# qq456cvb/CPPF

Measured on AMD Instinct MI355X. Metric: point-pairs/sec (PPF+MLP+vote+argmax), N=4096 K=128; 1/2/4/8 GPU, higher is better.
Workload: dtype f32; 1 GPU; c2: single object N=4096 K=128 (P=524288 pairs), bottle config, res 0.004, grid 26x76x26, num_rots 72 adaptive, fused PPF+MLP(MFMA f32)+decode of the  ... (full text: bench_full.json); parallelism=objects x1

## Files before the change

### cppf_amd/csrc/pair_mlp.hip

```cpp
#include <hip/hip_runtime.h>
#include <stdint.h>
#include <string.h>

#include "../../include/cppf.h"
#include "cppf_math.h"

using namespace cppf;

typedef float f32x4 __attribute__((ext_vector_type(4)));
typedef float f32x2 __attribute__((ext_vector_type(2)));
typedef float f32x4u __attribute__((ext_vector_type(4), aligned(4)));

#define CPPF_CHECK_LAUNCH()                         \
    do {                                            \
        hipError_t e__ = hipGetLastError();         \
        if (e__ != hipSuccess) return (int)e__;     \
    } while (0)

#include "pair_layout.h"

static bool is_std(int F, const int* dims, int n_res, int out_dim)
{
    return F == STD_F && n_res == 3 && dims[0] == 84 && dims[1] == 32 && dims[2] == 32 && dims[3] == 16 &&
           out_dim >= 1 && out_dim <= 16 * STD_NOB;
// ... 163 lines not shown
    if (__any(u < 0.f)) {
        asm volatile("" ::: "memory");
        int ak = 64;
#pragma unroll
        for (int k = NL - 1; k >= 0; --k)
            if (v[k] == mall) ak = k;
        const int am = NL * g + ak;
        int best = min(am, (int)xor16u((unsigned)am, lane));
        best = min(best, (int)xor32u((unsigned)best, lane));
        if (u < 0.f) { bin = best; owner = am == best; }
    }
    return owner;
}

struct MlpArgs {
    const float* pc;
    const float* nrm;
    const float* feat;
    const void* idxs;
    const float* packed;
    const float* u_tr;
    const float* u_rot;
    const float* table;
    float* out;
    float* outputs;
    float* heads;
    int64_t P;
    int out_dim;
    int idx64;
    float vr0, vr1;
    const int32_t* sel;
    const int32_t* n_sel;
};

template <typename T>
__device__ __forceinline__ const T& at_off(const void* base, unsigned byte_off)
{
    return *reinterpret_cast<const T*>(static_cast<const char*>(base) + byte_off);
}
template <typename T>
__device__ __forceinline__ T& at_off(void* base, unsigned byte_off)
{
    return *reinterpret_cast<T*>(static_cast<char*>(base) + byte_off);
}
__device__ __forceinline__ f3 ld3o(const float* __restrict__ base, int i)
{
    const unsigned o = __umul24((unsigned)i, 12u);
    return {at_off<float>(base, o), at_off<float>(base + 1, o), at_off<float>(base + 2, o)};
}

template <bool SEL>
__device__ __forceinline__ unsigned pair_row(const MlpArgs& A, int slot, int Pn)
{
    const unsigned s = (unsigned)min(slot, Pn - 1);
    return SEL ? (unsigned)at_off<int>(A.sel, s * 4u) : s;
}

template <bool SEL>
__device__ __forceinline__ void load_pair_idx(const MlpArgs& A, int slot, int Pn, int& ia, int& ib)
{
    const unsigned p = pair_row<SEL>(A, slot, Pn);
    const unsigned o = p * (A.idx64 ? 16u : 8u);
    ia = at_off<int>(A.idxs, o);
    ib = at_off<int>(static_cast<const char*>(A.idxs) + (A.idx64 ? 8 : 4), o);
}

__device__ __forceinline__ float ppf_from(f3 pa, f3 pb, f3 na, f3 nb, int g)
{
    const f3 xy = sub3(pa, pb);
    const float d = sqrt_rn((xy.x * xy.x + xy.y * xy.y) + xy.z * xy.z);
    const float den = d + 1e-7f;
    const float rden = refined_rcp(den);
    const f3 u = {div_by(xy.x, den, rden), div_by(xy.y, den, rden), div_by(xy.z, den, rden)};
    const float p0 = (na.x * u.x + na.y * u.y) + na.z * u.z;
    const float p1 = (nb.x * u.x + nb.y * u.y) + nb.z * u.z;
    const float p2 = (na.x * nb.x + na.y * nb.y) + na.z * nb.z;
    (void)g;
    const bool g0 = __builtin_amdgcn_inverse_ballot_w64(0x000000000000ffffull), g1 = __builtin_amdgcn_inverse_ballot_w64(0x00000000ffff0000ull),
               g2 = __builtin_amdgcn_inverse_ballot_w64(0x0000ffff00000000ull);
    const float s23 = g2 ? p2 : d, s123 = g1 ? p1 : s23;
    return g0 ? p0 : s123;
}

#define PROJ_PPB 8
__device__ __forceinline__ void point_proj_body(const float* __restrict__ feat, const float* __restrict__ packed, float* __restrict__ T,
                                                int64_t N)
{
    __shared__ float f[PROJ_PPB][STD_F];
    const int half = threadIdx.x >> 7, r = threadIdx.x & 127;
    const int64_t n0 = (int64_t)blockIdx.x * PROJ_PPB;
    for (int i = threadIdx.x; i < PROJ_PPB * STD_F; i += 256) {
        const int64_t n = n0 + i / STD_F;
        f[i / STD_F][i % STD_F] = n < N ? feat[n * STD_F + i % STD_F] : 0.f;
    }
    __syncthreads();
    float acc[PROJ_PPB / 2];
    const float b = r < 64 ? packed[OFF_BPT + r] : 0.f;
#pragma unroll
    for (int q = 0; q < PROJ_PPB / 2; ++q) acc[q] = b;
#pragma unroll 8
    for (int k = 0; k < STD_F; ++k) {
        const float w = packed[OFF_WPT + k * PROJ_COLS + r];
#pragma unroll
        for (int q = 0; q < PROJ_PPB / 2; ++q) acc[q] = fmaf(w, f[half + 2 * q][k], acc[q]);
    }
#pragma unroll
    for (int q = 0; q < PROJ_PPB / 2; ++q) {
        const int64_t n = n0 + half + 2 * q;
        if (n < N) T[n * PROJ_COLS + r] = acc[q];
    }
}
__global__ __launch_bounds__(256) void point_proj_kernel(const float* __restrict__ feat, const float* __restrict__ packed,
                                                         float* __restrict__ T, int64_t N)
{
    point_proj_body(feat, packed, T, N);
}
struct ProjBatch { const float* feat[8]; const float* packed[8]; float* table[8]; int64_t N[8]; };
__global__ __launch_bounds__(256) void point_proj_batch_kernel(ProjBatch B)
{
    const int i = blockIdx.y;
    if ((int64_t)blockIdx.x * PROJ_PPB >= B.N[i]) return;
    point_proj_body(B.feat[i], B.packed[i], B.table[i], B.N[i]);
}

template <bool LOGITS, bool DECODE, bool HEADS, bool SEL>
__device__ __forceinline__ void pair_mlp_body(const MlpArgs& A, const int wg, const int n_wg)
{
    extern __shared__ __attribute__((aligned(16))) float W[];
    {
        const f32x4* src = reinterpret_cast<const f32x4*>(A.packed);
        f32x4* dst = reinterpret_cast<f32x4*>(W);
        for (int k = threadIdx.x; k < STD_LDS / 4; k += MLP_THREADS) {
            int from = k;
            if (DECODE && k >= OFF_WF / 4 && k < OFF_B0B / 4) from = OFF_WFD / 4 + (k - OFF_WF / 4);
            if (DECODE && k >= OFF_BF / 4) from = OFF_BFD / 4 + (k - OFF_BF / 4);
            dst[k] = src[from];
        }
    }
    float* lut = W + STD_LDS;
    int* tile_ctr = reinterpret_cast<int*>(W + STD_LDS + 112);
    if (threadIdx.x == 0) *tile_ctr = 0;
    if (DECODE && threadIdx.x < 100) {
        const int k = threadIdx.x;
        float v;
        if (k < 32) v = ((float)k / 31.0f * 2.0f) * A.vr0 - A.vr0;
        else if (k < 64) v = (float)(k - 32) / 31.0f * A.vr1;
        else v = (float)(k - 64) / 35.0f * (float)CPPF_PI;
        lut[k] = v;
    }
    __syncthreads();

    const int lane = threadIdx.x & 63;
    const int j = lane & 15, g = lane >> 4;
    __builtin_assume(g >= 0 && g < 4);
    int Pn = (int)A.P;
    if (SEL) Pn = min(max(*A.n_sel, 0), Pn);
    const int n_tiles = (Pn + 16 * PB - 1) / (16 * PB);
    const int per_wg = (n_tiles + n_wg - 1) / n_wg;
    const int wg_begin = wg * per_wg;
    const int wg_end = min(wg_begin + per_wg, n_tiles);
    auto claim = [&]() -> int {
        int v = 0;
        if (lane == 0) v = atomicAdd(tile_ctr, 1);
        return wg_begin + __builtin_amdgcn_readfirstlane(v);
    };
    int cur = claim();
    if (cur >= wg_end) return;
    int nxt = claim();

    f32x4 acc[PB][4];
    int ia1[PB], ib1[PB];
    {
        f32x4 ta[PB][4], tb[PB][4];
        float xp[PB];
        int ia[PB], ib[PB];
#pragma unroll
        for (int pb = 0; pb < PB; ++pb) load_pair_idx<SEL>(A, cur * (16 * PB) + pb * 16 + j, Pn, ia[pb], ib[pb]);
#pragma unroll
        for (int pb = 0; pb < PB; ++pb) {
            const unsigned oa = (unsigned)ia[pb] * (PROJ_COLS * 4u) + 16u * g, ob_ = (unsigned)ib[pb] * (PROJ_COLS * 4u) + 256u + 16u * g;
#pragma unroll
            for (int ob = 0; ob < 4; ++ob) { ta[pb][ob] = at_off<f32x4>(A.table, oa + 64u * ob); tb[pb][ob] = at_off<f32x4>(A.table, ob_ + 64u * ob); }
            xp[pb] = ppf_from(ld3o(A.pc, ia[pb]), ld3o(A.pc, ib[pb]), ld3o(A.nrm, ia[pb]), ld3o(A.nrm, ib[pb]), g);
        }
        const int nt = nxt < wg_end ? nxt : cur;
#pragma unroll
        for (int pb = 0; pb < PB; ++pb) load_pair_idx<SEL>(A, nt * (16 * PB) + pb * 16 + j, Pn, ia1[pb], ib1[pb]);
// ... 654 lines not shown
```

### cppf_amd/csrc/vote.hip

```cpp
#include "vote_common.h"

#define VOTE_MAX_TILES 64
#define VOTE_WIN 72

__host__ __device__ inline int vote_fixed_bits_of(int64_t chunk_pairs, int n_rots)
{
    const double cap = 2048.0 * 4294967296.0 / ((double)(chunk_pairs > 0 ? chunk_pairs : 1) * n_rots) - 4.0;
    int kk = 24;
    while (kk > 8 && (double)(1u << kk) > cap) --kk;
    return kk;
}


static int v3_fixed_bits_bound(int64_t n_ppfs, int n_rots, int gx, int gy, int gz);
static bool v3_eligible(int64_t n_ppfs, int n_rots, int gx, int gy, int gz);
static size_t v3_workspace_bytes(int64_t n_ppfs, int gx, int gy, int gz);
static size_t v3_workspace_bytes_dyn(int many_tiles, int64_t n_ppfs);
static int v3_fused_tiles();
extern "C" int cppf_vote_fixed_point_bits(int64_t n_ppfs, int n_rots, int gx, int gy, int gz)
{
    if (n_rots < 1 || n_rots > CPPF_MAX_ROTS || gx < 1 || gy < 1 || gz < 1 || n_ppfs < 0) return -1;
    return v3_eligible(n_ppfs, n_rots, gx, gy, gz) ? v3_fixed_bits_bound(n_ppfs, n_rots, gx, gy, gz) : 0;
}

// ... 1056 lines not shown
            }
            while (qn >= 64 || (!more && qn > 0)) {
                const int take = qn < 64 ? qn : 64;
                __builtin_amdgcn_fence(__ATOMIC_ACQ_REL, "wavefront");
                const uint32_t off = lane < take ? pairq[qn - take + lane] : 0u;
                qn -= take;
                process(p0 + off, lane < take, 0u, 0u);
            }
            if (!more) break;
        }
    }

#ifdef V3_TRACE
    if (lane == 0) { trace[8 + wave] = wall_clock64(); unsigned hw; asm volatile("s_getreg_b32 %0, hwreg(HW_REG_HW_ID)" : "=s"(hw)); if (wave < 8) trace[24 + wave] = hw; }
#endif
    __syncthreads();
#ifdef V3_TRACE
    if (tid == 0) { trace[2] = wall_clock64(); trace[4] = (unsigned long long)t; trace[5] = (unsigned long long)c; trace[6] = (unsigned long long)ctrl[8]; trace[7] = (unsigned long long)ctrl[9]; }
#endif
    const int slot = v3_slot_words(pt, gz);
    uint4* part4 = reinterpret_cast<uint4*>(A.partials + (int64_t)bid * slot);
    const uint4* t4 = reinterpret_cast<const uint4*>(tile);
    for (int k = tid; k < (nwords + 3) >> 2; k += V3_THREADS) part4[k] = t4[k];
    bool wrote = false;
    auto to_plane = [&](const int w, const int lx, const int ly, const int z) {
        const uint32_t v = tile[w];
        if (v == 0u) return;
        unsigned long long* dst = &A.plane[((int64_t)(x0 + lx) * gy + (y0 + ly)) * gz + z];
        if (S > 0.f) atomicAdd(dst, (unsigned long long)v); else atomicAdd(reinterpret_cast<float*>(dst), __uint_as_float(v));
        wrote = true;
    };
    if (pt.hx && x0 + tx < gx)
        for (int k = tid; k < (ty + 1) * gz && k < ltyz; k += V3_THREADS) { const int ly = k / gz; to_plane(tx * ltyz + k, tx, ly, k - ly * gz); }
    if (pt.hy && y0 + ty < gy)
        for (int k = tid; k < tx * gz; k += V3_THREADS) { const int lx = k / gz, z = k - lx * gz; to_plane(lx * ltyz + ty * gz + z, lx, ty, z); }
    if (S > 0.f) {
        const int nc = min(ctrl[0], VOTE_CARRY_CAP);
        if (ctrl[0] > VOTE_CARRY_CAP && tid == 0) atomicOr(&A.hdr->flags, 1u);
        for (int k = tid; k < nc; k += V3_THREADS) {
            const int w = (int)carry_log[k];
            const int lx = w / ltyz, rem = w - lx * ltyz, ly = rem / gz, z = rem - ly * gz;
            atomicAdd(&A.plane[((int64_t)(x0 + lx) * gy + (y0 + ly)) * gz + z], 1ull << 32);
            wrote = true;
        }
    }
    if (__any(wrote) && lane == 0) A.hdr->any_extra = 1u;
#ifdef V3_TRACE
    __syncthreads();
    if (tid == 0) trace[3] = wall_clock64();
#endif
}

template <bool FUSED, bool WIDE>
__global__ __launch_bounds__(V3_THREADS) void v3_vote_kernel(V3Args A)
{
    v3_vote_body<FUSED, WIDE>(A, (int)blockIdx.x);
}

#define V3_BATCH_MAX 8
struct V3Batch {
    V3Args item[V3_BATCH_MAX];
    int wg_begin[V3_BATCH_MAX + 1];
    int red_begin[V3_BATCH_MAX + 1];
    int bps[V3_BATCH_MAX];
    int n;
};
static_assert(sizeof(V3Batch) <= 4096, "V3Batch travels by value: kernel arguments are limited to 4 KB");
__global__ __launch_bounds__(V3_THREADS) void v3_vote_batch_kernel(V3Batch B)
{
    int i = 0;
    while (i + 1 < B.n && (int)blockIdx.x >= B.wg_begin[i + 1]) ++i;
    if (B.item[i].fused) v3_vote_body<true, false>(B.item[i], (int)blockIdx.x - B.wg_begin[i]);
    else v3_vote_body<false, false>(B.item[i], (int)blockIdx.x - B.wg_begin[i]);
}

__device__ __forceinline__ void v3_rezero(V3Hdr* h)
{
    for (int k = 0; k < VOTE_MAX_TILES; ++k) h->tile_count[k * V3_CNT_STRIDE] = 0u;
    for (int k = 0; k < V3_RED_FANIN; ++k)
        for (int w = 2; w < 6; ++w) h->tile_count[k * V3_CNT_STRIDE + w] = 0u;
    h->flags = 0u; h->any_extra = 0u; h->done = 0u; h->magic = V3_MAGIC;
    __threadfence();
}
__device__ __forceinline__ void v3_reduce_body(const V3Args& A, const int bps, const int bid, const int nblocks)
{
    __shared__ unsigned long long part[RED_GROUPS][RED_CELLS];
    __shared__ unsigned long long wkey[RED_GROUPS];
    __shared__ int sp[200];
    const int tid = threadIdx.x, lane = tid & 63, cg = tid >> 6;
    if (bid == 0 && tid == 0) {
        const unsigned long long st = A.packed[31];
        if ((st & ~0xfffull) == VOTE_TAB_PENDING) A.packed[31] = st ^ (VOTE_TAB_PENDING ^ VOTE_TAB_STAMP);
    }
    int gx, gy, gz;
    int64_t n_points;
    V3Tiling pt;
    const bool fits = v3_resolve(A, gx, gy, gz, n_points, pt);
    const unsigned hflags = A.hdr->flags, hextra = A.hdr->any_extra, hfmt = A.hdr->fmt, hmagic = A.hdr->magic;
    const float hquantum = A.hdr->quantum;
    if (fits) v3_split(A, pt.T, sp);
    if (!fits || (hflags & 1u)) {
        const bool poisoned = hmagic != 0u && hmagic != V3_MAGIC;
        if (!poisoned) {
            uint4* p4 = reinterpret_cast<uint4*>(A.plane);
            const int64_t n16 = (int64_t)(V3_PLANE_BYTES / 16);
            for (int64_t i = (int64_t)bid * blockDim.x + tid; i < n16; i += (int64_t)nblocks * blockDim.x) p4[i] = make_uint4(0u, 0u, 0u, 0u);
            __threadfence();
            __syncthreads();
        }
        if (tid == 0) {
            const unsigned tk = atomicAdd(reinterpret_cast<unsigned*>(A.packed + 18), 1u);
            if (tk == (unsigned)nblocks - 1u) {
                if (A.out_idx) *A.out_idx = -1;
                if (A.out_val) *A.out_val = __uint_as_float(0x7fc00000u);
                if (A.quantum_out) *A.quantum_out = 0.f;
                A.packed[20] = 1ull;
                if (!poisoned) v3_rezero(A.hdr);
            }
        }
        return;
    }
    const bool earlier_pass_failed = A.win_base > 0 && A.packed[20] != 0ull;
    if (A.quantum_out && bid == 0 && tid == 0) *A.quantum_out = (hfmt == 0u && !earlier_pass_failed) ? hquantum : 0.f;
    const int T = pt.T;
    const int slot = v3_slot_words(pt, gz);
    __syncthreads();
    const bool raw = hfmt == 0u;
    const bool any_extra = hextra != 0u;
    unsigned long long best = 0ull;
    const bool wave_items = !A.fused && A.wgs <= 128;
    if (wave_items) {
        for (int item = bid * RED_GROUPS + cg; item < T * bps; item += nblocks * RED_GROUPS) {
            const int t = item / bps, j = item - t * bps;
            const int tix = t / pt.nty, tiy = t - tix * pt.nty;
            const int x0 = tix * pt.tx, y0 = tiy * pt.ty;
            const int tx = min(pt.tx, gx - x0), ty = min(pt.ty, gy - y0);
            const int tyh = pt.ty + pt.hy, ltyz = tyh * gz;
            const int nwords = (tx + pt.hx) * ltyz;
            const int k0 = j * RED_CELLS + lane * 4;
            if (k0 >= nwords) continue;
            const int C = sp[t], base_b = sp[64 + t];
            const unsigned n_own = (unsigned)sp[128 + t];
            unsigned long long acc[4] = {0ull, 0ull, 0ull, 0ull};
            float facc[4] = {0.f, 0.f, 0.f, 0.f};
            const uint32_t* base = A.partials + (int64_t)base_b * slot + k0;
            auto add = [&](const uint4 v) {
                if (raw) { acc[0] += v.x; acc[1] += v.y; acc[2] += v.z; acc[3] += v.w; }
                else { facc[0] += __uint_as_float(v.x); facc[1] += __uint_as_float(v.y); facc[2] += __uint_as_float(v.z); facc[3] += __uint_as_float(v.w); }
            };
            const bool full = n_own >= 64u * (unsigned)C;
            int c = 0;
            if (full) {
                for (; c + 3 < C; c += 4) {
                    uint4 v[4];
#pragma unroll
                    for (int q = 0; q < 4; ++q) v[q] = *reinterpret_cast<const uint4*>(base + (int64_t)(c + q) * slot);
#pragma unroll
                    for (int q = 0; q < 4; ++q) add(v[q]);
                }
            }
            for (; c < C; ++c)
                if (full || v3_chunk_live(n_own, c, C, base_b + c)) add(*reinterpret_cast<const uint4*>(base + (int64_t)c * slot));
#pragma unroll
            for (int u = 0; u < 4; ++u) {
                const int k = k0 + u;
                if (k >= nwords) continue;
                const int lx = k / ltyz, rem = k - lx * ltyz, ly = rem / gz, z = rem - ly * gz;
                if (!(lx < tx && ly < ty)) continue;
                const int64_t cell = ((int64_t)(x0 + lx) * gy + (y0 + ly)) * gz + z;
                const unsigned long long ext = any_extra ? A.plane[cell] : 0ull;
                if (ext) A.plane[cell] = 0ull;
                float v;
                if (raw) {
                    const unsigned long long s_ = ext + acc[u];
                    if (A.grid_raw) A.grid_raw[cell] = (long long)s_ + (A.accumulate ? A.grid_raw[cell] : 0ll);
                    v = (float)((double)s_ * (double)hquantum);
                } else {
                    v = __uint_as_float((uint32_t)ext) + facc[u];
                }
                if (A.accumulate && A.grid) v = A.grid[cell] + v;
                if (A.grid) A.grid[cell] = v;
                const unsigned long long key = ((unsigned long long)f2ord(v) << 32) | (unsigned long long)(0xffffffffu - (uint32_t)cell);
                best = key > best ? key : best;
            }
        }
    } else
    for (int item = bid; item < T * bps; item += nblocks) {
    const int t = item / bps, j = item - t * bps;
    const int tix = t / pt.nty, tiy = t - tix * pt.nty;
    const int x0 = tix * pt.tx, y0 = tiy * pt.ty;
    const int tx = min(pt.tx, gx - x0), ty = min(pt.ty, gy - y0);
    const int tyh = pt.ty + pt.hy, ltyz = tyh * gz;
    const int nwords = (tx + pt.hx) * ltyz;
    if (j * RED_CELLS >= nwords) continue;
    const int C = sp[t], base_b = sp[64 + t];
    const unsigned n_own = (unsigned)sp[128 + t];

    const int k0 = j * RED_CELLS + lane * 4;
    unsigned long long acc[4] = {0ull, 0ull, 0ull, 0ull};
    float facc[4] = {0.f, 0.f, 0.f, 0.f};
    if (k0 < nwords) {
        const uint32_t* base = A.partials + (int64_t)base_b * slot + k0;
        auto add = [&](const uint4 v) {
            if (raw) { acc[0] += v.x; acc[1] += v.y; acc[2] += v.z; acc[3] += v.w; }
            else { facc[0] += __uint_as_float(v.x); facc[1] += __uint_as_float(v.y); facc[2] += __uint_as_float(v.z); facc[3] += __uint_as_float(v.w); }
        };
        const int64_t cp = 64;
        const bool full = A.fused ? (int64_t)(C - 1) * cp < A.n_ppfs : n_own >= 64u * (unsigned)C;
        int c = cg;
        if (full) {
            for (; c + 7 * RED_GROUPS < C; c += 8 * RED_GROUPS) {
                uint4 v[8];
#pragma unroll
                for (int q = 0; q < 8; ++q) v[q] = *reinterpret_cast<const uint4*>(base + (int64_t)(c + q * RED_GROUPS) * slot);
#pragma unroll
                for (int q = 0; q < 8; ++q) add(v[q]);
            }
        }
        for (; c < C; c += RED_GROUPS)
            if (full || (A.fused ? (base_b + c == 0 || (int64_t)c * cp < A.n_ppfs) : v3_chunk_live(n_own, c, C, base_b + c)))
                add(*reinterpret_cast<const uint4*>(base + (int64_t)c * slot));
    }
#pragma unroll
    for (int u = 0; u < 4; ++u) part[cg][lane * 4 + u] = raw ? acc[u] : (unsigned long long)__float_as_uint(facc[u]);

    const int k = j * RED_CELLS + tid;
    int lx = 0, ly = 0, z = 0;
    bool owned = false;
    if (tid < RED_CELLS && k < nwords) {
        lx = k / ltyz;
        const int rem = k - lx * ltyz;
        ly = rem / gz; z = rem - ly * gz;
        owned = lx < tx && ly < ty;
    }
    const int64_t cell = ((int64_t)(x0 + lx) * gy + (y0 + ly)) * gz + z;
    unsigned long long ext = 0ull;
    float prev = 0.f;
    if (owned && any_extra) ext = A.plane[cell];
    if (owned && A.accumulate && A.grid) prev = A.grid[cell];
    __syncthreads();
    if (owned) {
        float v;
        if (ext) A.plane[cell] = 0ull;
        if (raw) {
            unsigned long long s_ = ext;
#pragma unroll
            for (int g = 0; g < RED_GROUPS; ++g) s_ += part[g][tid];
            if (A.grid_raw) A.grid_raw[cell] = (long long)s_ + (A.accumulate ? A.grid_raw[cell] : 0ll);
            v = (float)((double)s_ * (double)hquantum);
        } else {
            v = __uint_as_float((uint32_t)ext);
#pragma unroll
            for (int g = 0; g < RED_GROUPS; ++g) v = v + __uint_as_float((uint32_t)part[g][tid]);
        }
        if (A.accumulate) v = prev + v;
        if (A.grid) A.grid[cell] = v;
        const unsigned long long key = ((unsigned long long)f2ord(v) << 32) | (unsigned long long)(0xffffffffu - (uint32_t)cell);
        best = key > best ? key : best;
    }
    __syncthreads();
    }
    unsigned long long key = best;
    const int n_wkeys = wave_items ? RED_GROUPS : RED_CELLS / 64;
    if (cg < n_wkeys) {
        key = wave_max_u64(key);
        if (lane == 0) wkey[cg] = key;
    }
    const unsigned gsel = (unsigned)bid & (V3_RED_FANIN - 1);
    const unsigned n_group = ((unsigned)nblocks - gsel + V3_RED_FANIN - 1) / V3_RED_FANIN;
    const unsigned n_groups_used = (unsigned)nblocks < V3_RED_FANIN ? (unsigned)nblocks : V3_RED_FANIN;
    __syncthreads();
    if (tid == 0) {
        for (int w = 1; w < n_wkeys; ++w) key = wkey[w] > key ? wkey[w] : key;
        auto report = [](unsigned long long* slot_, unsigned long long k_) -> unsigned {
            const unsigned long long old = atomicMax(slot_, k_);
            unsigned d1 = (unsigned)old, d2;
            asm volatile("v_mov_b32 %0, %1" : "=v"(d2) : "v"(d1));
            return atomicAdd(reinterpret_cast<unsigned*>(slot_ + 1), 1u + (d1 ^ d2));
        };
        unsigned long long* gslot = reinterpret_cast<unsigned long long*>(&A.hdr->tile_count[gsel * V3_CNT_STRIDE + 2]);
        if (report(gslot, key) == n_group - 1) {
            const unsigned long long gbest = atomicMax(gslot, 0ull);
            if (report(A.packed, gbest) == n_groups_used - 1) {
                const unsigned long long best_all = atomicMax(A.packed, 0ull);
                if (A.out_idx) *A.out_idx = earlier_pass_failed ? -1ll : (long long)(0xffffffffu - (uint32_t)(best_all & 0xffffffffull));
                if (A.out_val) *A.out_val = earlier_pass_failed ? __uint_as_float(0x7fc00000u) : ord2f((uint32_t)(best_all >> 32));
                v3_rezero(A.hdr);
            }
        }
    }
}

__global__ __launch_bounds__(64 * RED_GROUPS) void v3_reduce_kernel(V3Args A, int bps)
{
    v3_reduce_body(A, bps, (int)blockIdx.x, (int)gridDim.x);
}
__global__ __launch_bounds__(64 * RED_GROUPS) void v3_reduce_batch_kernel(V3Batch B)
{
    int i = 0;
    while (i + 1 < B.n && (int)blockIdx.x >= B.red_begin[i + 1]) ++i;
    v3_reduce_body(B.item[i], B.bps[i], (int)blockIdx.x - B.red_begin[i], B.red_begin[i + 1] - B.red_begin[i]);
}

extern "C" size_t cppf_vote_workspace_init_bytes(void)
{
    return VOTE_WS_PART + V3_HDR_BYTES + V3_PLANE_BYTES;
}

static bool v3_eligible(int64_t n_ppfs, int n_rots, int gx, int gy, int gz)
{
    (void)n_rots;
    if (n_ppfs < 1 || n_ppfs > 0xffffffffll) return false;
    return v3_tiling(gx, gy, gz).T <= VOTE_MAX_TILES;
}
static int v3_fixed_bits_bound(int64_t n_ppfs, int n_rots, int gx, int gy, int gz)
{
    const V3Tiling t = v3_tiling(gx, gy, gz);
    const int wgs = v3_wgs(n_ppfs, t.T);
    if (t.T < v3_fused_tiles()) return v3_bits((unsigned)v3_fused_bits_pairs(n_ppfs, wgs / t.T, t.T), n_rots);
    const int wref = wgs < V3_BITS_WGS ? wgs : V3_BITS_WGS;
    const int64_t E = wref - t.T;
    const int64_t worst = E > 0 ? min(n_ppfs, (n_ppfs * t.T + E - 1) / E + 1) : n_ppfs;
    return v3_bits((unsigned)(worst > 0x7fffffff ? 0x7fffffff : worst), n_rots);
}
static size_t v3_workspace_bytes(int64_t n_ppfs, int gx, int gy, int gz)
{
    const V3Tiling t = v3_tiling(gx, gy, gz);
    return v3_plan(n_ppfs, t, gz, v3_wgs(n_ppfs, t.T), t.T < 4 ? 0 : n_ppfs, (int64_t)gx * gy * gz).total;
}
static inline int v3_dyn_tcap(int many_tiles)
{
    return many_tiles == 0 ? 3 : (many_tiles < 4 || many_tiles > VOTE_MAX_TILES ? VOTE_MAX_TILES : many_tiles);
}
static size_t v3_workspace_bytes_dyn(int many_tiles, int64_t n_ppfs)
{
    const int t_cap = v3_dyn_tcap(many_tiles), wgs = V3_WGS;
    return VOTE_WS_PART + V3_HDR_BYTES + V3_PLANE_BYTES +
           (many_tiles ? align_up((size_t)t_cap * (size_t)n_ppfs * 12, 256) + align_up((size_t)n_ppfs * V3_FRAME_BYTES, 256) : 0) +
           (size_t)wgs * V3_TILE_FLOATS * sizeof(uint32_t);
}
extern "C" int cppf_vote_plan_query(int64_t n_ppfs, int n_rots, int gx, int gy, int gz, int32_t* out)
{
    if (!out || n_rots < 1 || n_rots > CPPF_MAX_ROTS || gx < 1 || gy < 1 || gz < 1 || n_ppfs < 0) return CPPF_EINVAL;
    for (int k = 0; k < 10; ++k) out[k] = 0;
    if (v3_eligible(n_ppfs, n_rots, gx, gy, gz)) {
        const V3Tiling t = v3_tiling(gx, gy, gz);
        int wgs = v3_wgs(n_ppfs, t.T);
        if (t.T < v3_fused_tiles()) wgs = (wgs / t.T) * t.T;
        const int o[10] = {t.T < v3_fused_tiles() ? 2 : 3, t.T, t.tx, t.ty, t.ntx, t.nty, t.hx, t.hy, wgs, v3_fixed_bits_bound(n_ppfs, n_rots, gx, gy, gz)};
        for (int k = 0; k < 10; ++k) out[k] = o[k];
        return 0;
    }
    return 0;
}

struct VoteExtras { long long* grid_raw; float* quantum_out; int fixed_bits; };

#define V3_FUSED_TILES 4
static int v3_fused_tiles()
{
    static int v = 0;
    if (v == 0) {
        const char* e = getenv("CPPF_FUSED_MAX_TILES");
        const int w = e ? atoi(e) : V3_FUSED_TILES;
        v = w < V3_FUSED_TILES ? V3_FUSED_TILES : (w > VOTE_MAX_TILES + 1 ? VOTE_MAX_TILES + 1 : w);
    }
    return v;
}

struct V3Launch { V3Args A; int red_blocks, bps; };

static int v3_prepare(V3Launch& Lc, const float* points, const float* outputs, const float* probs, const void* point_idxs, int idx_is_i64,
                      float* grid_obj, const float* corner, float res, int64_t n_points, int64_t n_ppfs, int n_rots, int gx, int gy,
                      int gz, int adaptive, int accumulate, bool want_argmax, long long* out_idx, float* out_val, void* workspace,
                      const int32_t* shape_dev, int64_t grid_cap, int many_tiles, const VoteExtras* ex, int wg_cap, int wg_floor = V3_BITS_WGS)
{
    const int wgs_max = wg_cap > 0 ? (wg_cap < wg_floor ? wg_floor : (wg_cap > V3_WGS ? V3_WGS : wg_cap)) : V3_WGS;
    char* ws = static_cast<char*>(workspace);
    V3Args& A = Lc.A;
    A = V3Args{};
    if (ex) { A.grid_raw = ex->grid_raw; A.quantum_out = ex->quantum_out; A.kk_force = ex->fixed_bits; }
    A.points = points; A.outputs = outputs; A.probs = probs; A.point_idxs = point_idxs; A.idx64 = idx_is_i64;
    A.corner = corner; A.res = res; A.n_ppfs = n_ppfs; A.n_points = n_points; A.n_rots = n_rots; A.adaptive = adaptive;
    A.gx = gx; A.gy = gy; A.gz = gz; A.shape = shape_dev; A.grid_cap = grid_cap;
// ... 16 lines not shown
        A.partials = reinterpret_cast<uint32_t*>(A.frames) + (many_tiles ? align_up((size_t)n_ppfs * V3_FRAME_BYTES, 256) / 4 : 0);
        const int bps = ((V3_TILE_FLOATS + RED_CELLS - 1) / RED_CELLS + RED_FANIN - 1) / RED_FANIN * RED_FANIN;
        Lc.red_blocks = A.t_cap * bps;
    } else {
        A.t = v3_tiling(gx, gy, gz);
        A.wgs = v3_wgs(n_ppfs, A.t.T);
        if (A.wgs > wgs_max) A.wgs = wgs_max > A.t.T ? wgs_max : A.t.T;
        A.fused = A.t.T < v3_fused_tiles() ? 1 : 0;
        if (A.fused) {
            A.wgs = (A.wgs / A.t.T) * A.t.T;
            A.kk = v3_bits((unsigned)v3_fused_bits_pairs(n_ppfs, A.wgs / A.t.T, A.t.T), n_rots);
        }
        A.t_cap = A.t.T;
        const V3Plan pl = v3_plan(n_ppfs, A.t, gz, v3_wgs(n_ppfs, A.t.T), A.fused ? 0 : n_ppfs, (int64_t)gx * gy * gz);
        A.pool = reinterpret_cast<uint32_t*>(ws + pl.pool_off);
        A.frames = reinterpret_cast<float4*>(ws + pl.frames_off);
        A.partials = reinterpret_cast<uint32_t*>(ws + pl.part_off);
        const int bps = ((pl.slot + RED_CELLS - 1) / RED_CELLS + RED_FANIN - 1) / RED_FANIN * RED_FANIN;
        Lc.red_blocks = A.t.T * bps;
    }
    Lc.bps = Lc.red_blocks / A.t_cap;
    return 0;
}

static size_t v3_vote_lds(const V3Args& A) { return V3_LDS_HEAD + (size_t)(A.tab_entries + 2) * sizeof(float2) + (size_t)V3_TILE_FLOATS * sizeof(float); }
static void v3_set_attrs()
{
    static bool attr_done = false;
    if (!attr_done) {
        const void* ks[] = {reinterpret_cast<const void*>(&v3_bin_kernel<false>), reinterpret_cast<const void*>(&v3_bin_kernel<true>),
                            reinterpret_cast<const void*>(&v3_vote_kernel<false, false>), reinterpret_cast<const void*>(&v3_vote_kernel<true, false>),
                            reinterpret_cast<const void*>(&v3_vote_kernel<false, true>), reinterpret_cast<const void*>(&v3_vote_kernel<true, true>),
                            reinterpret_cast<const void*>(&v3_vote_batch_kernel)};
        for (const void* k : ks) (void)hipFuncSetAttribute(k, hipFuncAttributeMaxDynamicSharedMemorySize, 160 * 1024);
        attr_done = true;
    }
}

static size_t v3_bin_geometry(V3Args& A, dim3& bin_grid)
{
    int64_t srb = A.n_ppfs / ((int64_t)V3_BIN_THREADS * 512);
    srb = srb < 1 ? 1 : (srb > V3_BIN_SR ? V3_BIN_SR : srb);
    A.bin_sr = (int)srb;
    const int64_t rounds = (A.n_ppfs + V3_BIN_THREADS * srb - 1) / (V3_BIN_THREADS * srb);
    bin_grid = dim3((unsigned)(rounds < 512 ? rounds : 512));
    return (size_t)V3_STAGE * 16 + VOTE_BELOW_N * 16 + 2 * VOTE_MAX_TILES * 4 + 64 + (V3_BIN_THREADS / 64) * (V3_IRING * 2 + (64 * V3_BIN_SR + 64) * 4);
}

static int v3_launch(const float* points, const float* outputs, const float* probs, const void* point_idxs, int idx_is_i64,
                     float* grid_obj, const float* corner, float res, int64_t n_points, int64_t n_ppfs, int n_rots, int gx, int gy,
                     int gz, int adaptive, int accumulate, bool want_argmax, long long* out_idx, float* out_val, void* workspace,
                     hipStream_t st, const int32_t* shape_dev, int64_t grid_cap, int many_tiles, const VoteExtras* ex = nullptr,
                     int wg_cap = 0)
{
    V3Launch Lc;
    const int rc = v3_prepare(Lc, points, outputs, probs, point_idxs, idx_is_i64, grid_obj, corner, res, n_points, n_ppfs, n_rots, gx, gy, gz,
                              adaptive, accumulate, want_argmax, out_idx, out_val, workspace, shape_dev, grid_cap, many_tiles, ex, wg_cap);
    if (rc != 0) return rc;
    V3Args& A = Lc.A;
    const int red_blocks = Lc.red_blocks;
    const bool wide = n_rots > VOTE_WIN;
    v3_set_attrs();
    const size_t lds_vote = v3_vote_lds(A);
    dim3 bin_grid;
    const size_t lds_bin = v3_bin_geometry(A, bin_grid);
    const int bps = Lc.bps;
    const dim3 red_grid((unsigned)(red_blocks < 2 * V3_WGS ? red_blocks : 2 * V3_WGS));
    if (wide && A.grid_raw && !A.kk_force) A.kk_force = v3_fixed_bits_bound(n_ppfs, n_rots, gx, gy, gz);
    for (int wb = 0; wb < n_rots; wb += VOTE_WIN) {
        A.win_base = wb;
        if (wb > 0) A.accumulate = 1;
        if (A.fused) {
            if (wide) hipLaunchKernelGGL((v3_vote_kernel<true, true>), dim3((unsigned)A.wgs), dim3(V3_THREADS), lds_vote, st, A);
            else hipLaunchKernelGGL((v3_vote_kernel<true, false>), dim3((unsigned)A.wgs), dim3(V3_THREADS), lds_vote, st, A);
            CPPF_CHECK_LAUNCH();
        } else {
            if (wide) hipLaunchKernelGGL(v3_bin_kernel<true>, bin_grid, dim3(V3_BIN_THREADS), lds_bin, st, A);
            else hipLaunchKernelGGL(v3_bin_kernel<false>, bin_grid, dim3(V3_BIN_THREADS), lds_bin, st, A);
            CPPF_CHECK_LAUNCH();
            if (wide) hipLaunchKernelGGL((v3_vote_kernel<false, true>), dim3((unsigned)A.wgs), dim3(V3_THREADS), lds_vote, st, A);
            else hipLaunchKernelGGL((v3_vote_kernel<false, false>), dim3((unsigned)A.wgs), dim3(V3_THREADS), lds_vote, st, A);
            CPPF_CHECK_LAUNCH();
        }
        hipLaunchKernelGGL(v3_reduce_kernel, red_grid, dim3(64 * RED_GROUPS), 0, st, A, bps);
        CPPF_CHECK_LAUNCH();
    }
    return 0;
}

__global__ void zero_u64x2_kernel(unsigned long long* p) { p[0] = 0ull; p[1] = 0ull; }
__global__ void set_f32_kernel(float* p, float v) { *p = v; }

__global__ __launch_bounds__(256) void vote_global_kernel(const float* __restrict__ points, const float* __restrict__ outputs,
                                                          const float* __restrict__ probs, const void* __restrict__ point_idxs, int idx64,
                                                          float* __restrict__ grid, const float* __restrict__ corner, float res,
                                                          int64_t n_ppfs, int n_rots, int gx, int gy, int gz, int adaptive)
{
    const f3 cr = {corner[0], corner[1], corner[2]};
    const int64_t syz = (int64_t)gy * gz;
    for (int64_t p = (int64_t)blockIdx.x * blockDim.x + threadIdx.x; p < n_ppfs; p += (int64_t)gridDim.x * blockDim.x) {
        const float2 o = reinterpret_cast<const float2*>(outputs)[p];
        int2 ij;
        if (idx64) { const longlong2 v = reinterpret_cast<const longlong2*>(point_idxs)[p]; ij = make_int2((int)v.x, (int)v.y); }
        else ij = reinterpret_cast<const int2*>(point_idxs)[p];
        f3 a, ab, xd;
        if (!pair_frame(points, ij.x, ij.y, a, ab, xd)) continue;
        const f3 cc = sub3(a, scl3(ab, o.x));
        const float prob = probs ? fmaxf(probs[ij.x], probs[ij.y]) : 1.f;
        const f3 x = scl3(xd, o.y), y = cross3(x, ab);
        int n = n_rots;
        if (adaptive) n = min((int)((double)(o.y / res) * (2 * CPPF_PI)), n_rots);
        for (int i = 0; i < n; ++i) {
            const float2 cs = rot_cs(i, n);
            const f3 v = sub3(add3(cc, add3(scl3(x, cs.x), scl3(y, cs.y))), cr);
            const f3 g = {v.x / res, v.y / res, v.z / res};
            if ((double)g.x < 0.01 || (double)g.y < 0.01 || (double)g.z < 0.01 || (double)g.x >= (double)gx - 1.01 ||
                (double)g.y >= (double)gy - 1.01 || (double)g.z >= (double)gz - 1.01) continue;
            const int fx = (int)g.x, fy = (int)g.y, fz = (int)g.z;
            const float rx = g.x - floorf(g.x), ry = g.y - floorf(g.y), rz = g.z - floorf(g.z);
            const float w0x = 1.f - rx, w0y = 1.f - ry, w0z = 1.f - rz;
            float* b = grid + ((int64_t)fx * syz + (int64_t)fy * gz + fz);
            atomicAdd(b, w0x * w0y * w0z * prob);                 atomicAdd(b + 1, w0x * w0y * rz * prob);
            atomicAdd(b + gz, w0x * ry * w0z * prob);             atomicAdd(b + gz + 1, w0x * ry * rz * prob);
            atomicAdd(b + syz, rx * w0y * w0z * prob);            atomicAdd(b + syz + 1, rx * w0y * rz * prob);
            atomicAdd(b + syz + gz, rx * ry * w0z * prob);        atomicAdd(b + syz + gz + 1, rx * ry * rz * prob);
        }
    }
}

static int vote_impl(const float* points, const float* outputs, const float* probs, const void* point_idxs, int idx_is_i64,
                     float* grid_obj, const float* corner, float res, int64_t n_points, int64_t n_ppfs, int n_rots,
                     int gx, int gy, int gz, int adaptive, int accumulate, bool want_argmax, long long* out_idx, float* out_val,
                     void* workspace, size_t workspace_bytes, hipStream_t st, const int32_t* shape_dev = nullptr,
                     int64_t grid_cap = 0, int many_tiles = 0, const VoteExtras* ex = nullptr)
{
    const int wg_cap = (accumulate >> 8) & 0x1ff;
    if ((accumulate & ~(1 | (0x1ff << 8))) != 0) return CPPF_EINVAL;
    accumulate &= 1;
    if (wg_cap != 0 && ex) return CPPF_EINVAL;
    if (!points || (!grid_obj && !(ex && ex->grid_raw)) || !corner) return CPPF_EINVAL;
    if (n_ppfs > 0 && (!outputs || !point_idxs)) return CPPF_EINVAL;
    if (n_rots < 1 || n_rots > CPPF_MAX_ROTS || gx < 1 || gy < 1 || gz < 1 || n_ppfs < 0 || n_points < 1) return CPPF_EINVAL;
    if ((int64_t)gx * gy * gz > 0x7fffffffll) return CPPF_EINVAL;
    if (shape_dev) {
        if (n_ppfs < 1 || n_ppfs > 0xffffffffll || grid_cap < 1 || grid_cap > 0x7fffffffll) return CPPF_EINVAL;
        if (!workspace || workspace_bytes < v3_workspace_bytes_dyn(many_tiles, n_ppfs)) return CPPF_EWORKSPACE;
        return v3_launch(points, outputs, probs, point_idxs, idx_is_i64, grid_obj, corner, res, n_points, n_ppfs, n_rots, gx, gy, gz,
                         adaptive, accumulate, want_argmax, out_idx, out_val, workspace, st, shape_dev, grid_cap, many_tiles, ex, wg_cap);
    }
    if (v3_eligible(n_ppfs, n_rots, gx, gy, gz)) {
        if (!workspace || workspace_bytes < v3_workspace_bytes(n_ppfs, gx, gy, gz)) return CPPF_EWORKSPACE;
        return v3_launch(points, outputs, probs, point_idxs, idx_is_i64, grid_obj, corner, res, n_points, n_ppfs, n_rots, gx, gy, gz,
                         adaptive, accumulate, want_argmax, out_idx, out_val, workspace, st, nullptr, 0, 0, ex, wg_cap);
    }
    if (ex) {
        if (n_ppfs > 0) return CPPF_EUNSUPPORTED;
        if (!accumulate) {
            hipError_t e = hipMemsetAsync(ex->grid_raw, 0, (size_t)gx * gy * gz * sizeof(long long), st);
            if (e != hipSuccess) return (int)e;
        }
        hipLaunchKernelGGL(set_f32_kernel, dim3(1), dim3(1), 0, st, ex->quantum_out, HUGE_VALF);
        CPPF_CHECK_LAUNCH();
        return 0;
    }
    if (!workspace || workspace_bytes < 256) return CPPF_EWORKSPACE;
    const int64_t G = (int64_t)gx * gy * gz;
    if (!accumulate) {
// ... 3 lines not shown
    if (n_ppfs > 0) {
        int64_t nb = (n_ppfs + 255) / 256;
        if (nb > 4096) nb = 4096;
        hipLaunchKernelGGL(vote_global_kernel, dim3((unsigned)nb), dim3(256), 0, st, points, outputs, probs, point_idxs, idx_is_i64, grid_obj,
                           corner, res, n_ppfs, n_rots, gx, gy, gz, adaptive);
        CPPF_CHECK_LAUNCH();
    }
    if (want_argmax) {
        unsigned long long* packed = static_cast<unsigned long long*>(workspace);
        hipLaunchKernelGGL(zero_u64x2_kernel, dim3(1), dim3(1), 0, st, packed);
        int64_t nb = (G + 63) / 64;
        if (nb > RED_MAX_BLOCKS) nb = RED_MAX_BLOCKS;
        hipLaunchKernelGGL(reduce_argmax_kernel, dim3((unsigned)nb), dim3(64 * RED_GROUPS), 0, st, grid_obj, (const float*)nullptr, 0, G,
                           packed, 1, 0, out_idx, out_val);
        CPPF_CHECK_LAUNCH();
    }
    return 0;
}

extern "C" int cppf_ppf_voting(const float* points, const float* outputs, const float* probs,
                               const int32_t* point_idxs, float* grid_obj, const float* corner, float res,
                               int64_t n_points, int64_t n_ppfs, int n_rots, int gx, int gy, int gz, int adaptive,
                               void* workspace, size_t workspace_bytes, void* stream)
{
    return vote_impl(points, outputs, probs, point_idxs, 0, grid_obj, corner, res, n_points, n_ppfs, n_rots, gx, gy, gz,
                     adaptive, 1, false, nullptr, nullptr, workspace, workspace_bytes, (hipStream_t)stream);
}

extern "C" int cppf_vote_argmax(const float* points, const float* outputs, const float* probs,
                                const void* point_idxs, int idx_is_i64, float* grid_obj, const float* corner, float res,
                                int64_t n_points, int64_t n_ppfs, int n_rots, int gx, int gy, int gz, int adaptive,
                                int accumulate, long long* out_idx, float* out_val, void* workspace,
                                size_t workspace_bytes, void* stream)
{
    return vote_impl(points, outputs, probs, point_idxs, idx_is_i64, grid_obj, corner, res, n_points, n_ppfs, n_rots, gx, gy, gz,
                     adaptive, accumulate, true, out_idx, out_val, workspace, workspace_bytes, (hipStream_t)stream);
}

extern "C" int cppf_vote_argmax_dyn(const float* points, const float* outputs, const float* probs, const void* point_idxs,
                                    int idx_is_i64, float* grid_obj, int64_t grid_capacity, const float* corner, float res,
                                    int64_t n_points_cap, int64_t n_ppfs, int n_rots, const int32_t* shape_dev, int many_tiles,
                                    int adaptive, int accumulate, long long* out_idx, float* out_val, void* workspace,
                                    size_t workspace_bytes, void* stream)
{
    if (!shape_dev) return CPPF_EINVAL;
    return vote_impl(points, outputs, probs, point_idxs, idx_is_i64, grid_obj, corner, res, n_points_cap, n_ppfs, n_rots, 1, 1, 1,
                     adaptive, accumulate, true, out_idx, out_val, workspace, workspace_bytes, (hipStream_t)stream, shape_dev,
                     grid_capacity, many_tiles);
}

extern "C" int cppf_vote_batch_workgroups(int n_items, int flags)
{
    if (n_items < 1 || n_items > V3_BATCH_MAX) return CPPF_EINVAL;
    const int wg_cap = (flags >> 8) & 0x1ff;
    int w = wg_cap > 0 ? wg_cap : V3_WGS / n_items;
    if (w < V3_BITS_WGS) w = V3_BITS_WGS;
    if (w > V3_WGS) w = V3_WGS;
    return w;
}

extern "C" int cppf_vote_argmax_batch(int n_items, const CppfVoteItem* items, int n_rots, int adaptive, int flags, void* stream)
{
    if (n_items < 1 || n_items > V3_BATCH_MAX || !items) return CPPF_EINVAL;
    if ((flags & ~(1 | (0x1ff << 8))) != 0) return CPPF_EINVAL;
    if (n_rots < 1 || n_rots > CPPF_MAX_ROTS) return CPPF_EINVAL;
    hipStream_t st = (hipStream_t)stream;
    const int accumulate = flags & 1;
    auto shares_the_launch = [&](const CppfVoteItem& it) -> bool {
        const bool dyn = it.shape_dev != nullptr;
        bool batched = n_rots <= VOTE_WIN && it.n_ppfs >= 1 && it.points && it.grid && it.corner && it.outputs && it.point_idxs &&
                       it.out_idx && it.out_val && it.workspace && it.n_points >= 1;
        if (batched && dyn) batched = it.n_ppfs <= 0xffffffffll && it.grid_capacity >= 1 &&
                                      it.grid_capacity <= (int64_t)v3_dyn_tcap(it.many_tiles) * V3_TILE_FLOATS &&
                                      it.workspace_bytes >= v3_workspace_bytes_dyn(it.many_tiles, it.n_ppfs);
        if (batched && !dyn) batched = it.gx >= 1 && it.gy >= 1 && it.gz >= 1 && v3_eligible(it.n_ppfs, n_rots, it.gx, it.gy, it.gz) &&
                                       it.workspace_bytes >= v3_workspace_bytes(it.n_ppfs, it.gx, it.gy, it.gz);
        return batched;
    };
    int n_shared = 0;
    for (int i = 0; i < n_items; ++i) n_shared += shares_the_launch(items[i]) ? 1 : 0;
    const int width = cppf_vote_batch_workgroups(n_shared > 0 ? n_shared : n_items, flags);
    V3Batch B = {};
    int vote_wgs = 0, red_blocks = 0;
    size_t lds_vote = 0;
    for (int i = 0; i < n_items; ++i) {
        const CppfVoteItem& it = items[i];
        const bool dyn = it.shape_dev != nullptr;
        const bool batched = shares_the_launch(it);
        if (!batched) {
            const int rc = dyn ? cppf_vote_argmax_dyn(it.points, it.outputs, it.probs, it.point_idxs, it.idx_is_i64, it.grid, it.grid_capacity,
                                                      it.corner, it.res, it.n_points, it.n_ppfs, n_rots, it.shape_dev, it.many_tiles, adaptive,
                                                      flags, it.out_idx, it.out_val, it.workspace, it.workspace_bytes, stream)
                               : cppf_vote_argmax(it.points, it.outputs, it.probs, it.point_idxs, it.idx_is_i64, it.grid, it.corner, it.res,
                                                  it.n_points, it.n_ppfs, n_rots, it.gx, it.gy, it.gz, adaptive, flags, it.out_idx, it.out_val,
                                                  it.workspace, it.workspace_bytes, stream);
            if (rc != 0) return rc;
            continue;
        }
        V3Launch Lc;
        const int rc = v3_prepare(Lc, it.points, it.outputs, it.probs, it.point_idxs, it.idx_is_i64, it.grid, it.corner, it.res, it.n_points,
                                  it.n_ppfs, n_rots, dyn ? 1 : it.gx, dyn ? 1 : it.gy, dyn ? 1 : it.gz, adaptive, accumulate, true, it.out_idx,
                                  it.out_val, it.workspace, it.shape_dev, dyn ? it.grid_capacity : 0, dyn ? it.many_tiles : 0, nullptr, width);
        if (rc != 0) return rc;
        if (!Lc.A.fused) {
            v3_set_attrs();
            dim3 bin_grid;
            const size_t lds_bin = v3_bin_geometry(Lc.A, bin_grid);
            hipLaunchKernelGGL(v3_bin_kernel<false>, bin_grid, dim3(V3_BIN_THREADS), lds_bin, st, Lc.A);
            CPPF_CHECK_LAUNCH();
        }
        const int k = B.n++;
        B.item[k] = Lc.A;
        B.bps[k] = Lc.bps;
        B.wg_begin[k] = vote_wgs;
        B.red_begin[k] = red_blocks;
        vote_wgs += Lc.A.wgs;
        int rb = 2 * V3_WGS / (n_shared > 0 ? n_shared : n_items);
        rb = rb < 64 ? 64 : rb;
        if (!Lc.A.fused && rb < V3_WGS) rb = V3_WGS;
        red_blocks += Lc.red_blocks < rb ? Lc.red_blocks : rb;
        lds_vote = v3_vote_lds(Lc.A);
    }
    if (B.n == 0) return 0;
    B.wg_begin[B.n] = vote_wgs;
    B.red_begin[B.n] = red_blocks;
    v3_set_attrs();
    hipLaunchKernelGGL(v3_vote_batch_kernel, dim3((unsigned)vote_wgs), dim3(V3_THREADS), lds_vote, st, B);
    CPPF_CHECK_LAUNCH();
    hipLaunchKernelGGL(v3_reduce_batch_kernel, dim3((unsigned)red_blocks), dim3(64 * RED_GROUPS), 0, st, B);
    CPPF_CHECK_LAUNCH();
    return 0;
}

extern "C" int cppf_vote_grid_raw(const float* points, const float* outputs, const float* probs, const void* point_idxs,
                                  int idx_is_i64, long long* grid_raw, float* quantum_out, const float* corner, float res,
                                  int64_t n_points, int64_t n_ppfs, int n_rots, int gx, int gy, int gz, int adaptive, int accumulate,
                                  int fixed_bits, void* workspace, size_t workspace_bytes, void* stream)
{
    if (!grid_raw || !quantum_out || fixed_bits < 0 || (fixed_bits != 0 && (fixed_bits < 8 || fixed_bits > 24))) return CPPF_EINVAL;
    const VoteExtras ex = {grid_raw, quantum_out, fixed_bits};
    return vote_impl(points, outputs, probs, point_idxs, idx_is_i64, nullptr, corner, res, n_points, n_ppfs, n_rots, gx, gy, gz,
                     adaptive, accumulate, false, nullptr, nullptr, workspace, workspace_bytes, (hipStream_t)stream, nullptr, 0, 0, &ex);
}

__global__ __launch_bounds__(256) void grid_from_raw_kernel(const long long* __restrict__ raw, int64_t n, const float* __restrict__ quantum,
                                                            float* __restrict__ grid)
{
    const float q = *quantum;
    for (int64_t i = (int64_t)blockIdx.x * blockDim.x + threadIdx.x; i < n; i += (int64_t)gridDim.x * blockDim.x)
        grid[i] = (q > 0.f && q < INFINITY) ? (float)((double)raw[i] * (double)q)
                                            : (q > 0.f && raw[i] == 0ll ? 0.f : __uint_as_float(0x7fc00000u));
}
extern "C" int cppf_grid_from_raw(const long long* grid_raw, int64_t n, const float* quantum, float* grid, long long* out_idx,
                                  float* out_val, void* workspace, size_t workspace_bytes, void* stream)
{
    if (!grid_raw || !quantum || !grid || n < 1 || n > 0x7fffffffll) return CPPF_EINVAL;
    int64_t nb = (n + 255) / 256;
    hipLaunchKernelGGL(grid_from_raw_kernel, dim3((unsigned)(nb > 2048 ? 2048 : nb)), dim3(256), 0, (hipStream_t)stream, grid_raw, n, quantum, grid);
    CPPF_CHECK_LAUNCH();
    return out_idx ? cppf_grid_argmax(grid, n, out_idx, out_val, workspace, workspace_bytes, stream) : 0;
}

extern "C" int cppf_vote_tile_cells(void) { return V3_TILE_FLOATS; }

extern "C" int cppf_vote_tiles(int gx, int gy, int gz)
{
    if (gx < 1 || gy < 1 || gz < 1) return CPPF_EINVAL;
    const int T = v3_tiling(gx, gy, gz).T;
    return T <= VOTE_MAX_TILES ? T : 0;
}

extern "C" int cppf_grid_argmax(const float* grid, int64_t n, long long* out_idx, float* out_val, void* workspace,
                                size_t workspace_bytes, void* stream)
{
    if (!grid || n < 1 || n > 0x7fffffffll || !out_idx) return CPPF_EINVAL;
    if (!workspace || workspace_bytes < 16) return CPPF_EWORKSPACE;
    hipStream_t st = (hipStream_t)stream;
    unsigned long long* packed = static_cast<unsigned long long*>(workspace);
    hipLaunchKernelGGL(zero_u64x2_kernel, dim3(1), dim3(1), 0, st, packed);
    int64_t nb = (n + 63) / 64;
    if (nb > RED_MAX_BLOCKS) nb = RED_MAX_BLOCKS;
    hipLaunchKernelGGL(reduce_argmax_kernel, dim3((unsigned)nb), dim3(64 * RED_GROUPS), 0, st, const_cast<float*>(grid),
                       (const float*)nullptr, 0, n, packed, 1, 0, out_idx, out_val);
    CPPF_CHECK_LAUNCH();
    return 0;
}

extern "C" int cppf_abi_version(void) { return CPPF_ABI_VERSION; }
extern "C" const char* cppf_error_string(int code)
{
    switch (code) {
    case 0: return "success";
    case CPPF_EINVAL: return "cppf: invalid argument";
    case CPPF_EWORKSPACE: return "cppf: workspace missing or too small";
    case CPPF_EUNSUPPORTED: return "cppf: unsupported layer shape";
    case CPPF_ENONFINITE: return "cppf: the cloud holds non-finite coordinates";
    case CPPF_ECAPACITY: return "cppf: a device-side bound (bin list capacity) was exceeded";
    default: return code > 0 ? hipGetErrorString((hipError_t)code) : "cppf: unknown error";
    }
}
```

Baseline: 6.609 billion pairs/s.

## Add lean software-pipelined vote reduce path and register-cached point projection weights

The vote reduce kernel gains a LEAN template variant for fused, shape-free votes with few chunks per tile. It prefetches two work items' partial sums, plane extras and previous grid values into registers before the loop and issues the next loads right after consuming the current ones, so global latency overlaps with the LDS reduction. It also raises the occupancy hint. Separately, the point projection caches its weight column in registers, reads LDS features as float4 and handles 16 points per block instead of 8. Costs are higher register pressure and duplicated reduce logic that must stay consistent with the existing path.

```diff
diff --git a/cppf_amd/csrc/pair_mlp.hip b/cppf_amd/csrc/pair_mlp.hip
--- a/cppf_amd/csrc/pair_mlp.hip
+++ b/cppf_amd/csrc/pair_mlp.hip
@@ -269,27 +269,36 @@
     return g0 ? p0 : s123;
 }
 
-#define PROJ_PPB 8
+#define PROJ_PPB 16
+static_assert(STD_F % 4 == 0, "the feature rows are read from LDS as float4");
 __device__ __forceinline__ void point_proj_body(const float* __restrict__ feat, const float* __restrict__ packed, float* __restrict__ T,
                                                 int64_t N)
 {
-    __shared__ float f[PROJ_PPB][STD_F];
+    __shared__ __attribute__((aligned(16))) float f[PROJ_PPB][STD_F];
     const int half = threadIdx.x >> 7, r = threadIdx.x & 127;
     const int64_t n0 = (int64_t)blockIdx.x * PROJ_PPB;
+    float w[STD_F];
+#pragma unroll
+    for (int k = 0; k < STD_F; ++k) w[k] = packed[OFF_WPT + k * PROJ_COLS + r];
+    const float b = r < 64 ? packed[OFF_BPT + r] : 0.f;
     for (int i = threadIdx.x; i < PROJ_PPB * STD_F; i += 256) {
         const int64_t n = n0 + i / STD_F;
         f[i / STD_F][i % STD_F] = n < N ? feat[n * STD_F + i % STD_F] : 0.f;
     }
     __syncthreads();
     float acc[PROJ_PPB / 2];
-    const float b = r < 64 ? packed[OFF_BPT + r] : 0.f;
 #pragma unroll
     for (int q = 0; q < PROJ_PPB / 2; ++q) acc[q] = b;
-#pragma unroll 8
-    for (int k = 0; k < STD_F; ++k) {
-        const float w = packed[OFF_WPT + k * PROJ_COLS + r];
-#pragma unroll
-        for (int q = 0; q < PROJ_PPB / 2; ++q) acc[q] = fmaf(w, f[half + 2 * q][k], acc[q]);
+#pragma unroll
+    for (int k = 0; k < STD_F; k += 4) {
+#pragma unroll
+        for (int q = 0; q < PROJ_PPB / 2; ++q) {
+            const float4 x = *reinterpret_cast<const float4*>(&f[half + 2 * q][k]);
+            acc[q] = fmaf(w[k], x.x, acc[q]);
+            acc[q] = fmaf(w[k + 1], x.y, acc[q]);
+            acc[q] = fmaf(w[k + 2], x.z, acc[q]);
+            acc[q] = fmaf(w[k + 3], x.w, acc[q]);
+        }
     }
 #pragma unroll
     for (int q = 0; q < PROJ_PPB / 2; ++q) {
diff --git a/cppf_amd/csrc/vote.hip b/cppf_amd/csrc/vote.hip
--- a/cppf_amd/csrc/vote.hip
+++ b/cppf_amd/csrc/vote.hip
@@ -1162,22 +1162,62 @@
     h->flags = 0u; h->any_extra = 0u; h->done = 0u; h->magic = V3_MAGIC;
     __threadfence();
 }
+template <bool LEAN>
 __device__ __forceinline__ void v3_reduce_body(const V3Args& A, const int bps, const int bid, const int nblocks)
 {
     __shared__ unsigned long long part[RED_GROUPS][RED_CELLS];
     __shared__ unsigned long long wkey[RED_GROUPS];
     __shared__ int sp[200];
     const int tid = threadIdx.x, lane = tid & 63, cg = tid >> 6;
-    if (bid == 0 && tid == 0) {
-        const unsigned long long st = A.packed[31];
-        if ((st & ~0xfffull) == VOTE_TAB_PENDING) A.packed[31] = st ^ (VOTE_TAB_PENDING ^ VOTE_TAB_STAMP);
-    }
+    const bool stamper = bid == 0 && tid == 0;
+    const unsigned long long tab_st = stamper ? A.packed[31] : 0ull;
+    const unsigned hflags = A.hdr->flags, hextra = A.hdr->any_extra, hfmt = A.hdr->fmt, hmagic = A.hdr->magic;
+    const float hquantum = A.hdr->quantum;
     int gx, gy, gz;
     int64_t n_points;
     V3Tiling pt;
     const bool fits = v3_resolve(A, gx, gy, gz, n_points, pt);
-    const unsigned hflags = A.hdr->flags, hextra = A.hdr->any_extra, hfmt = A.hdr->fmt, hmagic = A.hdr->magic;
-    const float hquantum = A.hdr->quantum;
+    const int n_items = fits ? pt.T * bps : 0;
+    const int Cf = LEAN && fits ? A.wgs / pt.T : 0;
+    const int slot_f = fits ? v3_slot_words(pt, gz) : 0;
+    struct Pre { uint4 v[2]; unsigned long long ext; float prev; int cell; bool owned, any; };
+    Pre pq[2];
+    auto chunk_live = [&](int t, int c) { return c < Cf && (t * Cf + c == 0 || (int64_t)c * 64 < A.n_ppfs); };
+    auto issue = [&](int it0) {
+#pragma unroll
+        for (int u = 0; u < 2; ++u) {
+            Pre& q = pq[u];
+            q.v[0] = q.v[1] = make_uint4(0u, 0u, 0u, 0u);
+            q.ext = 0ull; q.prev = 0.f; q.cell = 0; q.owned = false; q.any = false;
+            const int item = it0 + u * nblocks;
+            if (item >= n_items) continue;
+            const int t = item / bps, j = item - t * bps;
+            const int tix = t / pt.nty, tiy = t - tix * pt.nty;
+            const int x0 = tix * pt.tx, y0 = tiy * pt.ty;
+            const int tx = min(pt.tx, gx - x0), ty = min(pt.ty, gy - y0);
+            const int ltyz = (pt.ty + pt.hy) * gz;
+            const int nwords = (tx + pt.hx) * ltyz;
+            if (j * RED_CELLS >= nwords) continue;
+            q.any = true;
+            const int k0 = j * RED_CELLS + lane * 4;
+            if (k0 < nwords) {
+                const uint32_t* base = A.partials + (int64_t)t * Cf * slot_f + k0;
+#pragma unroll
+                for (int s = 0; s < 2; ++s)
+                    if (chunk_live(t, cg + s * RED_GROUPS)) q.v[s] = *reinterpret_cast<const uint4*>(base + (int64_t)(cg + s * RED_GROUPS) * slot_f);
+            }
+            const int k = j * RED_CELLS + tid;
+            if (tid < RED_CELLS && k < nwords) {
+                const int lx = k / ltyz, rem = k - lx * ltyz, ly = rem / gz, z = rem - ly * gz;
+                q.owned = lx < tx && ly < ty;
+                q.cell = ((x0 + lx) * gy + (y0 + ly)) * gz + z;
+            }
+            if (q.owned) q.ext = A.plane[q.cell];
+            if (q.owned && A.accumulate && A.grid) q.prev = A.grid[q.cell];
+        }
+    };
+    if (LEAN) issue(bid);
+    if (stamper && (tab_st & ~0xfffull) == VOTE_TAB_PENDING) A.packed[31] = tab_st ^ (VOTE_TAB_PENDING ^ VOTE_TAB_STAMP);
     if (fits) v3_split(A, pt.T, sp);
     if (!fits || (hflags & 1u)) {
         const bool poisoned = hmagic != 0u && hmagic != V3_MAGIC;
@@ -1209,7 +1249,53 @@
     const bool any_extra = hextra != 0u;
     unsigned long long best = 0ull;
     const bool wave_items = !A.fused && A.wgs <= 128;
-    if (wave_items) {
+    if (LEAN) {
+        for (int it0 = bid;;) {
+#pragma unroll
+            for (int u = 0; u < 2; ++u) {
+                const Pre& q = pq[u];
+                if (!q.any) continue;
+                const int t = (it0 + u * nblocks) / bps;
+                unsigned long long acc[4] = {0ull, 0ull, 0ull, 0ull};
+                float facc[4] = {0.f, 0.f, 0.f, 0.f};
+#pragma unroll
+                for (int s = 0; s < 2; ++s) {
+                    if (!chunk_live(t, cg + s * RED_GROUPS)) continue;
+                    const uint4 v = q.v[s];
+                    if (raw) { acc[0] += v.x; acc[1] += v.y; acc[2] += v.z; acc[3] += v.w; }
+                    else { facc[0] += __uint_as_float(v.x); facc[1] += __uint_as_float(v.y); facc[2] += __uint_as_float(v.z); facc[3] += __uint_as_float(v.w); }
+                }
+#pragma unroll
+                for (int w = 0; w < 4; ++w) part[cg][lane * 4 + w] = raw ? acc[w] : (unsigned long long)__float_as_uint(facc[w]);
+                __syncthreads();
+                if (q.owned) {
+                    const int64_t cell = q.cell;
+                    const unsigned long long ext = any_extra ? q.ext : 0ull;
+                    float v;
+                    if (ext) A.plane[cell] = 0ull;
+                    if (raw) {
+                        unsigned long long s_ = ext;
+#pragma unroll 4
+                        for (int g = 0; g < RED_GROUPS; ++g) s_ += part[g][tid];
+                        if (A.grid_raw) A.grid_raw[cell] = (long long)s_ + (A.accumulate ? A.grid_raw[cell] : 0ll);
+                        v = (float)((double)s_ * (double)hquantum);
+                    } else {
+                        v = __uint_as_float((uint32_t)ext);
+#pragma unroll 4
+                        for (int g = 0; g < RED_GROUPS; ++g) v = v + __uint_as_float((uint32_t)part[g][tid]);
+                    }
+                    if (A.accumulate) v = q.prev + v;
+                    if (A.grid) A.grid[cell] = v;
+                    const unsigned long long key = ((unsigned long long)f2ord(v) << 32) | (unsigned long long)(0xffffffffu - (uint32_t)cell);
+                    best = key > best ? key : best;
+                }
+                __syncthreads();
+            }
+            it0 += 2 * nblocks;
+            if (it0 >= n_items) break;
+            issue(it0);
+        }
+    } else if (wave_items) {
         for (int item = bid * RED_GROUPS + cg; item < T * bps; item += nblocks * RED_GROUPS) {
             const int t = item / bps, j = item - t * bps;
             const int tix = t / pt.nty, tiy = t - tix * pt.nty;
@@ -1371,15 +1457,18 @@
     }
 }
 
-__global__ __launch_bounds__(64 * RED_GROUPS) void v3_reduce_kernel(V3Args A, int bps)
-{
-    v3_reduce_body(A, bps, (int)blockIdx.x, (int)gridDim.x);
-}
-__global__ __launch_bounds__(64 * RED_GROUPS) void v3_reduce_batch_kernel(V3Batch B)
+__host__ __device__ inline bool v3_red_lean(const V3Args& A) { return A.fused && !A.shape && A.wgs / A.t.T <= 2 * RED_GROUPS; }
+template <bool LEAN>
+__global__ __launch_bounds__(64 * RED_GROUPS, LEAN ? 8 : 4) void v3_reduce_kernel(V3Args A, int bps)
+{
+    v3_reduce_body<LEAN>(A, bps, (int)blockIdx.x, (int)gridDim.x);
+}
+template <bool LEAN>
+__global__ __launch_bounds__(64 * RED_GROUPS, LEAN ? 8 : 4) void v3_reduce_batch_kernel(V3Batch B)
 {
     int i = 0;
     while (i + 1 < B.n && (int)blockIdx.x >= B.red_begin[i + 1]) ++i;
-    v3_reduce_body(B.item[i], B.bps[i], (int)blockIdx.x - B.red_begin[i], B.red_begin[i + 1] - B.red_begin[i]);
+    v3_reduce_body<LEAN>(B.item[i], B.bps[i], (int)blockIdx.x - B.red_begin[i], B.red_begin[i + 1] - B.red_begin[i]);
 }
 
 extern "C" size_t cppf_vote_workspace_init_bytes(void)
@@ -1562,7 +1651,8 @@
             else hipLaunchKernelGGL((v3_vote_kernel<false, false>), dim3((unsigned)A.wgs), dim3(V3_THREADS), lds_vote, st, A);
             CPPF_CHECK_LAUNCH();
         }
-        hipLaunchKernelGGL(v3_reduce_kernel, red_grid, dim3(64 * RED_GROUPS), 0, st, A, bps);
+        if (v3_red_lean(A)) hipLaunchKernelGGL(v3_reduce_kernel<true>, red_grid, dim3(64 * RED_GROUPS), 0, st, A, bps);
+        else hipLaunchKernelGGL(v3_reduce_kernel<false>, red_grid, dim3(64 * RED_GROUPS), 0, st, A, bps);
         CPPF_CHECK_LAUNCH();
     }
     return 0;
@@ -1732,6 +1822,7 @@
     const int width = cppf_vote_batch_workgroups(n_shared > 0 ? n_shared : n_items, flags);
     V3Batch B = {};
     int vote_wgs = 0, red_blocks = 0;
+    bool lean = true;
     size_t lds_vote = 0;
     for (int i = 0; i < n_items; ++i) {
         const CppfVoteItem& it = items[i];
@@ -1760,6 +1851,7 @@
             CPPF_CHECK_LAUNCH();
         }
         const int k = B.n++;
+        lean = lean && v3_red_lean(Lc.A);
         B.item[k] = Lc.A;
         B.bps[k] = Lc.bps;
         B.wg_begin[k] = vote_wgs;
@@ -1777,7 +1869,8 @@
     v3_set_attrs();
     hipLaunchKernelGGL(v3_vote_batch_kernel, dim3((unsigned)vote_wgs), dim3(V3_THREADS), lds_vote, st, B);
     CPPF_CHECK_LAUNCH();
-    hipLaunchKernelGGL(v3_reduce_batch_kernel, dim3((unsigned)red_blocks), dim3(64 * RED_GROUPS), 0, st, B);
+    if (lean) hipLaunchKernelGGL(v3_reduce_batch_kernel<true>, dim3((unsigned)red_blocks), dim3(64 * RED_GROUPS), 0, st, B);
+    else hipLaunchKernelGGL(v3_reduce_batch_kernel<false>, dim3((unsigned)red_blocks), dim3(64 * RED_GROUPS), 0, st, B);
     CPPF_CHECK_LAUNCH();
     return 0;
 }
```

Result: slower. 6.410 billion pairs/s (-3.0%).
